# gbbin/DDP-practice

Hardware: AMD Instinct MI355X
Metric: images/sec (whole node) + 3-epoch wall-clock, MNIST ConvNet at 1/2/4/8 MI355X (higher is better)
Workload: dtype bf16; 1 GPU; model=ConvNet (2x[Conv5x5-BN-ReLU-MaxPool2] + Linear(1568,10), 29,034 params), global_batch=32, parallelism=dp1, per_rank_batch=32, impl=native (fused HIP kernels, C++ reducer/communicator), sync_bn=False, amp=autocast bf16 + GradScaler, optimizer=SGD(lr=1e-4), hipgraph=True, steps_per_graph=16, comm=none (1 rank), grad_avg=none (1 rank)

## Files before the change

### ddp_practice_amd/csrc/kernels/conv5x5.h

```cpp
#pragma once
#include "convblock_bn.h"

namespace dpa {
namespace cb {

template <int I> struct SH;
template <> struct SH<0> { static constexpr int CIN = 1, COUT = 16, H = 28, W = 28, SPLIT = 4, WROWS = 28; };
template <> struct SH<1> { static constexpr int CIN = 16, COUT = 32, H = 14, W = 14, SPLIT = 2, WROWS = 14; };

__host__ __device__ constexpr int conv5x5_win_rows(int H, int W, int nsplit, bool even) {
  const int HW = H * W, MT = (HW + 15) / 16;
  int mx = 0;
  for (int sp = 0; sp < nsplit; ++sp) {
    const int p0 = 16 * (MT * sp / nsplit), p1e = 16 * (MT * (sp + 1) / nsplit), p1 = p1e < HW ? p1e : HW;
    if (p1 <= p0) return 0;
    int lo = p0 / W - 2, hi = (p1 - 1) / W + 2;
    lo = lo < 0 ? 0 : lo;
    hi = hi > H - 1 ? H - 1 : hi;
    if (even) {
      lo &= ~1;
      hi |= 1;
    }
    mx = hi - lo + 1 > mx ? hi - lo + 1 : mx;
  }
  return mx;
}

template <typename T>
struct BwdEpi {
  const uint8_t* idx;
  const T* xh;
  float* bslab;
};

constexpr int W2F_ROWS = 32, W2F_PITCH = 424;
constexpr int W2D_ROWS = 16, W2D_PITCH = 808;
constexpr int W2F_LEN = W2F_ROWS * W2F_PITCH, W2D_LEN = W2D_ROWS * W2D_PITCH;
template <typename T>
struct WPack {
  const float* w2 = nullptr;
  T* fwd = nullptr;
  T* dgrad = nullptr;
};
template <typename T>
__device__ __forceinline__ void pack_w2(const WPack<T>& pk) {
  const int total = W2F_LEN + W2D_LEN;
  for (int e = blockIdx.x * blockDim.x + threadIdx.x; e < total; e += gridDim.x * blockDim.x) {
    if (e < W2F_LEN) {
      const int co = e / W2F_PITCH, k = e % W2F_PITCH;
      const float v = k < 400 ? pk.w2[(co * 16 + (k & 15)) * 25 + (k >> 4)] : 0.f;
      pk.fwd[e] = Cvt<T>::from_f(v);
    } else {
      const int e2 = e - W2F_LEN;
      const int ci = e2 / W2D_PITCH, k = e2 % W2D_PITCH;
      const float v = k < 800 ? pk.w2[((k & 31) * 16 + ci) * 25 + (24 - (k >> 5))] : 0.f;
      pk.dgrad[e2] = Cvt<T>::from_f(v);
    }
  }
}

struct GatherIn {
  const uint8_t* imgs = nullptr;
  const int64_t* labels = nullptr;
  const int64_t* order = nullptr;
  long long order_len = 0;
  int* ctr = nullptr;
  int64_t* lab_out = nullptr;
  float scale = 1.f, shift = 0.f;
  int nimg = 0;
};

template <typename T, int CIN, int H, int W>
__host__ __device__ constexpr size_t conv5x5_img_bytes() {
  return ((sizeof(T) * (size_t)(H + 4) * (W + 4) * CIN) + 15) / 16 * 16;
}
template <typename T, int CIN, int COUT, int H, int W>
__host__ __device__ constexpr size_t conv5x5_dyn_bytes() {
  return conv5x5_img_bytes<T, CIN, H, W>() + sizeof(T) * (size_t)COUT * (ceil_to(25 * CIN, 32) + 8);
}

template <typename T, int CIN, int COUT, int H, int W, int MODE, int PRO = 0, int EPI = 0, int WPK = 0,
          bool DYN = false, int WR = H>
__device__ __forceinline__ void
conv5x5_body(const T* __restrict__ x, const float* __restrict__ w, const float* __restrict__ bias,
             T* __restrict__ y, float* __restrict__ fslab, float* __restrict__ fstats,
             const float* __restrict__ shift, int nsplit, const PoolIn<T>& pin, const BwdIn<T>& bin,
             const BwdEpi<T>& epi, const T* __restrict__ wpk, const WPack<T>& pk, const int bid,
             const GatherIn& gin = GatherIn{}) {
  static_assert(CIN == 1 || CIN % 8 == 0, "CIN must be 1 or a multiple of 8");
  static_assert(COUT % 16 == 0, "COUT must be a multiple of 16");
  static_assert((H * W) % 4 == 0, "H*W must be a multiple of 4");
  static_assert(PRO != 2 || MODE == 2, "PRO 2 is a data-grad prologue");
  static_assert(PRO != 3 || (CIN == 1 && MODE != 2), "PRO 3 gathers single-channel input images");
  static_assert(EPI == 0 || MODE == 2, "EPI 1 is a data-grad epilogue");
  constexpr int NCH = CIN >= 8 ? CIN / 8 : 1;
  constexpr int HP = H + 4, WPD = W + 4;
  constexpr int K = 25 * CIN;
  constexpr int KP = ceil_to(K, 32);
  constexpr int KS = KP / 32;
  constexpr int KPW = KP + 8;
  constexpr int NT = COUT / 16;
  constexpr int HW = H * W;
  constexpr int MT = (HW + 15) / 16;
  typedef MM<T> mm;

  T* img;
  T* wl;
  if constexpr (DYN) {
    img = reinterpret_cast<T*>(dpa_dyn_lds);
    wl = reinterpret_cast<T*>(dpa_dyn_lds + conv5x5_img_bytes<T, CIN, H, W>());
  } else {
// ... 125 lines not shown
    }
  };
  auto store_epi = [&]() {
    if constexpr (EPI == 1) {
#pragma unroll
      for (int i = 0; i < EIT; ++i) {
        const int e = tid + i * NTHR;
        if (e < COUT * enp) {
          const int co = e / enp, pp = e % enp;
          eidx[co * EPIX + pp] = ei[i];
          exh[co * EPIX + pp] = ex[i];
        }
      }
    }
  };
  if constexpr (PRO != 2) {
    load_epi();
    store_epi();
  }
  DPA_STAMP(2);
  constexpr int DQ = PRO != 1 ? 1
                     : (CIN % 8 == 0 && sizeof(T) == 2) ? 8 * ((CIN / 8 * SR * W + NTHR - 1) / NTHR)
                                                          : (CIN * SR * W + NTHR - 1) / NTHR;
  int dq_e[DQ];
  T dq_p[DQ], dq_x[DQ];
  uint8_t dq_i[DQ];
#pragma unroll
  for (int d = 0; d < DQ; ++d) dq_e[d] = -1;
  if constexpr (PRO == 0) {
    stage_chw<T, CIN, H, W>(xb, [&](int ci, int h, int ww, T a, T bb) {
      img[imo((h + 2) * WPD + (ww + 2), ci)] = a;
      img[imo((h + 2) * WPD + (ww + 3), ci)] = bb;
    });
  } else if constexpr (PRO == 3) {
    static_assert(HW % 4 == 0 && W % 4 == 0, "4-pixel groups stay inside a row");
    constexpr int G4 = HW / 4, GIT = (G4 + NTHR - 1) / NTHR;
    const int step = __builtin_amdgcn_readfirstlane(*reinterpret_cast<volatile int*>(gin.ctr));
    long long pos = (long long)step * gin.nimg + b;
    pos = pos < gin.order_len ? pos : gin.order_len - 1;
    const int64_t src = gin.order[pos];
    const uint32_t* s4 = reinterpret_cast<const uint32_t*>(gin.imgs + src * HW);
    uint32_t v4[GIT];
#pragma unroll
    for (int i = 0; i < GIT; ++i)
      if (tid + i * NTHR < G4) v4[i] = s4[tid + i * NTHR];
    if (sp == 0 && tid == 0) gin.lab_out[b] = gin.labels[src];
// ... 31 lines not shown
    const bool wr = pin.p_out != nullptr;
    if constexpr (CIN % 8 == 0 && sizeof(T) == 2) {
      constexpr int NO = CIN / 8, NPI = NO * RP, IT8 = (NPI + NTHR - 1) / NTHR;
      P top[IT8][8], bot[IT8][8];
      auto ld8 = [&](int i, int o, int ho, int wo) {
#pragma unroll
        for (int j = 0; j < 8; ++j) {
          const P* src = reinterpret_cast<const P*>(yb + ((size_t)(8 * o + j) * 2 * H + 2 * ho) * 2 * W + 2 * wo);
          top[i][j] = src[0];
          bot[i][j] = src[W];
        }
      };
#pragma unroll
      for (int i = 0; i < IT8; ++i) {
        const int e8 = tid + i * NTHR;
        if constexpr (WIN) {
          const int ec = min(e8, NPI - 1);
          ld8(i, ec / RP, min(r_lo + (ec % RP) / W, H - 1), ec % W);
        } else if (e8 < NPI) {
          ld8(i, e8 / RP, (e8 % RP) / W, e8 % W);
        }
      }
      load_wpk();
      bn_finalize<CIN>(pin.bn, sc_s, beta_s, mean_s, istd_s, part, bid);
      DPA_STAMP(3);
#pragma unroll
      for (int i = 0; i < IT8; ++i) {
        const int e8 = tid + i * NTHR;
        const int o = e8 / RP, hl = (e8 % RP) / W, ho = r_lo + hl, wo = e8 % W;
        if (e8 < NPI && (!WIN || hl < r_n)) {
          const int pix = ho * W + wo;
          const bool own = wr && pix >= p_lo && pix < p_hi;
          unsigned pk[4];
#pragma unroll
          for (int j = 0; j < 8; ++j) {
            const int ci = 8 * o + j;
            float best, xh;
            int bi;
            bn_relu_max4x<T>(top[i][j], bot[i][j], sc_s[ci], beta_s[ci], mean_s[ci], istd_s[ci], best, bi, xh);
            const T pvj = Cvt<T>::from_f(best);
            const unsigned bits = __builtin_bit_cast(unsigned short, pvj);
            if (j & 1) pk[j >> 1] |= bits << 16; else pk[j >> 1] = bits;
            const int e = ci * HW + pix;
            const int d = i * 8 + j;
            dq_e[d] = own ? e : -1;
            dq_p[d] = pvj;
// ... 2 lines not shown
          }
          *reinterpret_cast<uint4*>(&img[imo((ho + 2) * WPD + (wo + 2), 8 * o)]) = make_uint4(pk[0], pk[1], pk[2], pk[3]);
        }
      }
    } else {
      constexpr int NPS = CIN * RP, IT = (NPS + NTHR - 1) / NTHR;
      P top[IT], bot[IT];
      auto ld1 = [&](int i, int ci, int ho, int wo) {
        const P* src = reinterpret_cast<const P*>(yb + ((size_t)ci * 2 * H + 2 * ho) * 2 * W + 2 * wo);
        top[i] = src[0];
        bot[i] = src[W];
      };
#pragma unroll
      for (int i = 0; i < IT; ++i) {
        const int e = tid + i * NTHR;
        if constexpr (WIN) {
          const int ec = min(e, NPS - 1);
          ld1(i, ec / RP, min(r_lo + (ec % RP) / W, H - 1), ec % W);
        } else if (e < NPS) {
          ld1(i, e / RP, (e % RP) / W, e % W);
        }
      }
      load_wpk();
      bn_finalize<CIN>(pin.bn, sc_s, beta_s, mean_s, istd_s, part, bid);
      DPA_STAMP(3);
#pragma unroll
      for (int i = 0; i < IT; ++i) {
        const int e = tid + i * NTHR;
        const int ci = e / RP, hl = (e % RP) / W, ho = r_lo + hl, wo = e % W;
        if (e < NPS && (!WIN || hl < r_n)) {
          const int pix = ho * W + wo;
          float best, xh;
          int bi;
          bn_relu_max4x<T>(top[i], bot[i], sc_s[ci], beta_s[ci], mean_s[ci], istd_s[ci], best, bi, xh);
          const T pv = Cvt<T>::from_f(best);
          img[imo((ho + 2) * WPD + (wo + 2), ci)] = pv;
          dq_e[i] = wr && pix >= p_lo && pix < p_hi ? ci * HW + pix : -1;
          dq_p[i] = pv;
          dq_i[i] = (uint8_t)(bi | (best > 0.f ? IDX_RELU : 0));
          dq_x[i] = Cvt<T>::from_f(xh);
        }
      }
    }
  } else {
    __shared__ float coef[5 * CIN], sums[2 * CIN];
    __shared__ float part[NTHR];
// ... 25 lines not shown
        if (WIN && h >= r_n) return;
        const int hp = r_lo + h + 2;
        img[imo(hp * WPD + (ww + 2), c)] = v00;
        img[imo(hp * WPD + (ww + 3), c)] = v01;
        img[imo((hp + 1) * WPD + (ww + 2), c)] = v10;
        img[imo((hp + 1) * WPD + (ww + 3), c)] = v11;
      });
    }
    store_epi();
  }
  DPA_STAMP(4);
  __syncthreads();
  DPA_STAMP(5);
  if constexpr (PRO == 1) {
    constexpr int NPO = CIN * HW;
#pragma unroll
    for (int d = 0; d < DQ; ++d)
      if (dq_e[d] >= 0) {
        const size_t o = (size_t)b * NPO + dq_e[d];
        pin.p_out[o] = dq_p[d];
        pin.idx_out[o] = dq_i[d];
        pin.xh_out[o] = dq_x[d];
      }
  }

  const int lane = tid & 63, wv = tid >> 6;
  const int r = lane & 15, q = lane >> 4;

  float s1[NT], s2[NT];
#pragma unroll
  for (int nt = 0; nt < NT; ++nt) s1[nt] = s2[nt] = 0.f;

  for (int mt = mt0 + wv; mt < mt1; mt += NTHR / 64) {
    const int m = mt * 16 + r;
    const int mm_ = m < HW ? m : HW - 1;
    const int oh = mm_ / W, ow = mm_ % W;
    f32x4 acc[NT];
#pragma unroll
    for (int nt = 0; nt < NT; ++nt) acc[nt] = f32x4{0.f, 0.f, 0.f, 0.f};
#pragma unroll
    for (int s = 0; s < KS; ++s) {
      typename mm::frag a;
      if constexpr (CIN == 1) {
#pragma unroll
        for (int j = 0; j < 8; ++j) {
          const int tap = 32 * s + 8 * q + j;
// ... 57 lines not shown
    if (tid < 2 * COUT) {
      float t = 0.f;
#pragma unroll
      for (int w2 = 0; w2 < NTHR / 64; ++w2) t += lstat[w2 * 2 * COUT + tid];
      row[tid] = t;
    }
    if constexpr (MODE == 0) {
      if (tid == 0) {
        const int p0 = mt0 * 16, p1 = min(mt1 * 16, HW);
        row[2 * COUT] = (float)(p1 - p0);
      }
      if (bid == 0 && tid < COUT) fstats[2 * COUT + 1 + tid] = shift[tid];
    }
  }
  DPA_STAMP(7);
}

template <typename T, int CIN, int COUT, int H, int W, int MODE, int PRO = 0, int EPI = 0, int WPK = 0, int WR = H>
__global__ void __launch_bounds__(NTHR)
conv5x5_kernel(const T* __restrict__ x, const float* __restrict__ w, const float* __restrict__ bias,
               T* __restrict__ y, float* __restrict__ fslab, float* __restrict__ fstats,
               const float* __restrict__ shift, int nsplit, PoolIn<T> pin = PoolIn<T>{},
               BwdIn<T> bin = BwdIn<T>{}, BwdEpi<T> epi = BwdEpi<T>{}, const T* __restrict__ wpk = nullptr,
               WPack<T> pk = WPack<T>{}, GatherIn gin = GatherIn{}) {
  conv5x5_body<T, CIN, COUT, H, W, MODE, PRO, EPI, WPK, false, WR>(x, w, bias, y, fslab, fstats, shift, nsplit, pin,
                                                                   bin, epi, wpk, pk, (int)blockIdx.x, gin);
}

}
}
```

### ddp_practice_amd/csrc/kernels/convnet_fused.hip

```cpp
#include <type_traits>

#include "conv5x5.h"
#include "conv5x5_wgrad.h"
#include "comm/xgmi.h"

namespace dpa {
namespace cnf {

using cb::BNParams;
using cb::bn_finalize;
using cb::bn_relu_max4x;
using cb::BwdEpi;
using cb::BwdIn;
using cb::IDX_POS;
using cb::IDX_RELU;
using cb::Pair2;
using cb::PoolIn;
using cb::with_t;

constexpr int HF = 256;
constexpr int NTHR_HB = 256;

template <typename T, int C, int H, int W, int NMAX>
__global__ void __launch_bounds__(HF)
// ... 175 lines not shown
  bi.dbeta = dbeta.has_value() ? dbeta->data_ptr<float>() : nullptr;
  return bi;
}

typedef std::shared_ptr<xgmi::XgmiComm> XcPtr;
static xgmi::XSite site_of(const XcPtr& xc, int s) { return xc ? xc->site(s) : xgmi::XSite{}; }

int64_t fwd2_split(bool fp32) { return fp32 ? cb::kFwd2SplitT<float> : cb::kFwd2SplitT<__half>; }

template <int NSPLIT, bool EVEN>
constexpr int conv2_wr() {
  constexpr int need = cb::conv5x5_win_rows(14, 14, NSPLIT, EVEN);
  static_assert(need > 0, "conv2: more workgroups per image than 16-pixel tiles");
  return need < 14 ? need : 14;
}
static void conv2_row_window(int wr, int nsplit, bool even, const char* what) {
  const int need = cb::conv5x5_win_rows(14, 14, nsplit, even);
  TORCH_CHECK(need > 0 && (wr >= 14 || need <= wr), what, ": a split in ", nsplit, " stages up to ", need,
              " rows, the kernel's window holds ", wr);
}
template <typename T>
constexpr int kFwd2WR = conv2_wr<cb::kFwd2SplitT<T>, false>();

void conv2_fwd(at::Tensor y1, c10::optional<at::Tensor> fslab1, at::Tensor fstats1, at::Tensor g1, at::Tensor b1,
               at::Tensor rm1, at::Tensor rv1, at::Tensor nbt1, double momentum, double eps, bool train, at::Tensor w2,
               at::Tensor bias2, at::Tensor y2, c10::optional<at::Tensor> fslab2, at::Tensor fstats2, at::Tensor rm2,
               c10::optional<at::Tensor> p1_out, c10::optional<at::Tensor> idx1_out,
               c10::optional<at::Tensor> xh1_out, at::Tensor wpk, XcPtr xc) {
  DPA_CHECK_INPUT(y1); DPA_CHECK_INPUT(w2); DPA_CHECK_INPUT(y2); DPA_CHECK_INPUT(wpk);
  TORCH_CHECK(wpk.numel() == cb::W2F_LEN && wpk.scalar_type() == y1.scalar_type(), "packed conv2 weights");
  const int B = (int)y1.size(0);
  TORCH_CHECK(y1.size(1) == 16 && y1.size(2) == 28 && y1.size(3) == 28 && w2.size(0) == 32 && w2.size(1) == 16,
              "fused conv2 expects the ConvNet shapes");
  TORCH_CHECK(y2.scalar_type() == y1.scalar_type());
  TORCH_CHECK(p1_out.has_value() == idx1_out.has_value() && p1_out.has_value() == xh1_out.has_value());
  if (p1_out.has_value())
    TORCH_CHECK(p1_out->numel() == (int64_t)B * 16 * 196 && idx1_out->numel() == p1_out->numel() &&
                xh1_out->numel() == p1_out->numel());
  const int ns = fwd2_split(y1.scalar_type() == at::kFloat);
  if (train) TORCH_CHECK(fslab2.has_value() && fslab2->numel() == (int64_t)B * ns * cb::fslab_row(32));
  if (B == 0) return;
  BNParams bp = bn_params(fslab1, fstats1, g1, b1, rm1, rv1, nbt1, momentum, eps, train, 16);
  if (train) {
    bp.xs = site_of(xc, xgmi::kSiteFwd1);
    xgmi::set_site_grid(bp.xs, B * ns, "conv2_fwd");
  }
  hipStream_t stream = cur_stream();
  with_t(dt_of(y1), [&](auto tag) {
    typedef decltype(tag) T;
    PoolIn<T> pin{dptr<T>(y1), bp, p1_out.has_value() ? dptr<T>(*p1_out) : nullptr,
                  idx1_out.has_value() ? idx1_out->data_ptr<uint8_t>() : nullptr,
                  xh1_out.has_value() ? dptr<T>(*xh1_out) : nullptr};
    constexpr int WR = kFwd2WR<T>;
    conv2_row_window(WR, ns, false, "conv2_fwd");
    if (train)
      hipLaunchKernelGGL((cb::conv5x5_kernel<T, 16, 32, 14, 14, 0, 1, 0, 1, WR>), dim3(B * ns), dim3(cb::NTHR), 0,
                         stream, nullptr, nullptr, bias2.data_ptr<float>(), dptr<T>(y2), fslab2->data_ptr<float>(),
                         fstats2.data_ptr<float>(), rm2.data_ptr<float>(), ns, pin, BwdIn<T>{}, BwdEpi<T>{},
                         dptr<T>(wpk), cb::WPack<T>{});
    else
      hipLaunchKernelGGL((cb::conv5x5_kernel<T, 16, 32, 14, 14, 1, 1, 0, 1, WR>), dim3(B * ns), dim3(cb::NTHR), 0,
                         stream, nullptr, nullptr, bias2.data_ptr<float>(), dptr<T>(y2), nullptr, nullptr, nullptr,
                         ns, pin, BwdIn<T>{}, BwdEpi<T>{}, dptr<T>(wpk), cb::WPack<T>{});
  });
  DPA_CHECK_LAUNCH();
}

void head_fwd(at::Tensor y2, c10::optional<at::Tensor> fslab2, at::Tensor fstats2, at::Tensor g2, at::Tensor b2,
              at::Tensor rm2, at::Tensor rv2, at::Tensor nbt2, double momentum, double eps, bool train, at::Tensor wfc,
              at::Tensor bfc, at::Tensor logits, c10::optional<at::Tensor> p2_out, c10::optional<at::Tensor> idx2_out,
              c10::optional<at::Tensor> xh2_out, XcPtr xc) {
  DPA_CHECK_INPUT(y2); DPA_CHECK_INPUT(wfc); DPA_CHECK_INPUT(logits);
  const int B = (int)y2.size(0), N = (int)wfc.size(0);
  TORCH_CHECK(y2.size(1) == 32 && y2.size(2) == 14 && y2.size(3) == 14 && wfc.size(1) == 32 * 49,
              "fused head expects the ConvNet shapes");
  TORCH_CHECK(N >= 1 && N <= 64, "fused head supports up to 64 classes");
  TORCH_CHECK(logits.numel() == (int64_t)B * N && logits.scalar_type() == y2.scalar_type());
  TORCH_CHECK(p2_out.has_value() == idx2_out.has_value() && p2_out.has_value() == xh2_out.has_value());
  if (p2_out.has_value())
    TORCH_CHECK(p2_out->numel() == (int64_t)B * 1568 && idx2_out->numel() == p2_out->numel() &&
                xh2_out->numel() == p2_out->numel());
  if (B == 0) return;
// ... 528 lines not shown
        B * fwd2_split(std::is_same<T, float>::value));
    ok = ok && co_resident(reinterpret_cast<const void*>(&head_fwd_kernel<T, 32, 14, 14, 16>), (int)B, HF, 0) &&
         co_resident(reinterpret_cast<const void*>(&head_fwd_kernel<T, 32, 14, 14, 64>), (int)B, HF, 0);
    chk(reinterpret_cast<const void*>(&cb::conv5x5_kernel<T, 32, 16, 14, 14, 2, 2, 1, 1, kDgrad2WR<T>>), B * kDgradSplitT<T>);
    if (conv2_bwd_dyn<T>())
      ok = ok && co_resident(reinterpret_cast<const void*>(&conv2_bwd_dyn_kernel<T>),
                             (int)(B * kDgradSplitT<T> + wgrad2_wgs(B) + FC_BLOCKS), cb::NTHR,
                             conv2_bwd_dyn_bytes<T>());
    else if constexpr (!std::is_same<T, float>::value)
      chk(reinterpret_cast<const void*>(&conv2_bwd_kernel<T>), B * kDgradSplitT<T> + wgrad2_wgs(B) + FC_BLOCKS);
    chk(reinterpret_cast<const void*>(&conv2_wgrad_kernel<T>), wgrad2_wgs(B));
    chk(reinterpret_cast<const void*>(&cb::conv5x5_wgrad_kernel<T, 1, 16, 28, 28, WG1_ROWS, 2>),
        wgrad_bn_rows(1, B));
    chk(reinterpret_cast<const void*>(&wgrad1_slab2_kernel<T>), wgrad_bn_rows(1, B));
  });
  return ok;
}

}

void register_convnet_fused(pybind11::module& m) {
  namespace py = pybind11;
  auto s = m.def_submodule("convnet", "whole-ConvNet fused kernels");
  s.def("conv2_fwd", &cnf::conv2_fwd);
  s.def("head_fwd", &cnf::head_fwd);
  s.def("head_bwd", &cnf::head_bwd);
  s.def("head_bwd_lds", &cnf::head_bwd_lds);
  s.def("dgrad2_rows", &cnf::dgrad2_rows, py::arg("B"), py::arg("fp32") = false);
  s.def("conv1_fwd_pack", &cnf::conv1_fwd_pack);
  s.def("conv1_fwd_pack_gather", &cnf::conv1_fwd_pack_gather);
#ifdef DPA_TIMING
  s.def("read_stamps", []() {
    auto out = at::empty({DPA_MAX_STAMP_BLOCKS, DPA_NSTAMPS}, at::TensorOptions().dtype(at::kLong));
    DPA_CHECK_HIP(hipDeviceSynchronize());
    DPA_CHECK_HIP(hipMemcpyFromSymbol(out.data_ptr(), HIP_SYMBOL(dpa_stamps), sizeof(unsigned long long) *
                                      DPA_MAX_STAMP_BLOCKS * DPA_NSTAMPS));
    return out;
  });
  s.def("clear_stamps", []() {
    DPA_CHECK_HIP(hipDeviceSynchronize());
    std::vector<unsigned long long> z(DPA_MAX_STAMP_BLOCKS * DPA_NSTAMPS, 0ull);
    DPA_CHECK_HIP(hipMemcpyToSymbol(HIP_SYMBOL(dpa_stamps), z.data(), z.size() * sizeof(unsigned long long)));
  });
#endif
  s.attr("W2F_LEN") = cb::W2F_LEN;
  s.attr("W2D_LEN") = cb::W2D_LEN;
  s.def("conv2_dgrad", &cnf::conv2_dgrad);
// ... 11 lines not shown
```

### ddp_practice_amd/csrc/kernels/convnet_head.hip

```cpp
#include <cstdlib>

#include "comm/xgmi.h"
#include "convblock_bn.h"

namespace dpa {
namespace cnh {

using cb::BNParams;
using cb::IDX_RELU;
using cb::Pair2;

constexpr int NT_MAX = 1024;
constexpr int C = 32, H = 14, W = 14, HO = 7, WO = 7, PP = 49, K = C * PP;
constexpr int BMAX = 64;
constexpr int NMAX = 16;

constexpr int kArrShift = 57, kBadShift = 50;
constexpr unsigned long long kSumMask = (1ull << kBadShift) - 1ull;
constexpr double kFix = 16777216.0;
constexpr float kRowMax = 1048575.f;

struct HeadRow {
  const int64_t* target;
  int64_t ignore_index;
  float smoothing;
  const float* scale;
  int has_scale;
  unsigned long long* state;
  float* loss;
  float* dlog;
  void* dls;
  void* dp2;
  float* bsum;
  int* chk;
};



template <typename T, int NM, int NT>
__global__ void __launch_bounds__(NT)
head_row_kernel(const T* __restrict__ y, BNParams bn, const float* __restrict__ wfc, const float* __restrict__ bfc,
                T* __restrict__ logits, T* __restrict__ p_out, uint8_t* __restrict__ idx_out,
                T* __restrict__ xh_out, int B, int N, HeadRow hr) {
  typedef typename Pair2<T>::type P;
  constexpr int IT = (K + NT - 1) / NT;
  constexpr int NW = NT / 64;
  constexpr int CL = NT / C;
  __shared__ float sc_s[C], beta_s[C], mean_s[C], istd_s[C];
  __shared__ float part_s[NT];
  __shared__ float red[NW][NM];
  __shared__ float lgs[NM];
  __shared__ float gs[2][IT * NT];

  const int tid = threadIdx.x, b = blockIdx.x;
  const int lane = tid & 63, wv = tid >> 6;

  DPA_STAMP(0);
  const T* yb = y + (size_t)b * C * H * W;
  P top[IT], bot[IT];
#pragma unroll
  for (int i = 0; i < IT; ++i) {
    const int k = min(tid + i * NT, K - 1);
    const int c = k / PP, j = k % PP, ho = j / WO, wo = j % WO;
    const P* src = reinterpret_cast<const P*>(yb + ((size_t)c * H + 2 * ho) * W + 2 * wo);
    top[i] = src[0];
    bot[i] = src[W / 2];
  }
  float wq[NM][IT];
#pragma unroll
  for (int n = 0; n < NM; ++n) {
    const float* wr = wfc + (size_t)min(n, N - 1) * K;
#pragma unroll
    for (int i = 0; i < IT; ++i) wq[n][i] = wr[min(tid + i * NT, K - 1)];
  }
  float bias[NM];
#pragma unroll
  for (int n = 0; n < NM; ++n) bias[n] = bfc[min(n, N - 1)];
  const int64_t tgt_lane = hr.target[min(lane, B - 1)];
  const int64_t tgt = hr.target[b];
  const float scv = hr.scale[0];
  DPA_STAMP(1);
  constexpr int RU = NT == 256 && cb::kFwd2SplitT<T> > 2 ? (32 * cb::kFwd2SplitT<T> + 2) / 3 : cb::RSUM_U;
  cb::bn_finalize<C, RU>(bn, sc_s, beta_s, mean_s, istd_s, part_s, b);
  DPA_STAMP(2);
  if (hr.chk != nullptr && b == 0 && tid == 0) {
    hr.chk[0] = 0;
    hr.chk[1] = __float_as_int(scv);
  }
  float pf[IT], xf[IT];
  uint8_t ixr[IT];
#pragma unroll
  for (int i = 0; i < IT; ++i) {
    const int k = tid + i * NT;
    const int c = min(k, K - 1) / PP;
    float best, xh;
    int bi;
    cb::bn_relu_max4x<T>(top[i], bot[i], sc_s[c], beta_s[c], mean_s[c], istd_s[c], best, bi, xh);
    const T pv = Cvt<T>::from_f(best);
    const T xq = Cvt<T>::from_f(xh);
    ixr[i] = (uint8_t)(bi | (best > 0.f ? IDX_RELU : 0));
    pf[i] = k < K ? Cvt<T>::to_f(pv) : 0.f;
    xf[i] = Cvt<T>::to_f(xq);
    if (k < K) {
      const size_t o = (size_t)b * K + k;
      p_out[o] = pv;
      idx_out[o] = ixr[i];
      xh_out[o] = xq;
    }
  }
#pragma unroll
  for (int n = 0; n < NM; ++n)
#pragma unroll
    for (int i = 0; i < IT; ++i) wq[n][i] = n < N ? rnd_t<T>(wq[n][i]) : 0.f;
#pragma unroll
  for (int n = 0; n < NM; ++n) {
    float a = 0.f;
#pragma unroll
    for (int i = 0; i < IT; ++i) a += pf[i] * wq[n][i];
    a = wave_sum_dpp(a);
    if (lane == 0) red[wv][n] = a;
  }
  lds_barrier();
  if (NW > 4) {
    if (tid < NM) {
      float t = 0.f;
#pragma unroll
      for (int n = 0; n < NM; ++n) t = tid == n ? bias[n] : t;
#pragma unroll
      for (int w = 0; w < NW; ++w) t += red[w][tid];
      lgs[tid] = t;
    }
    lds_barrier();
  }
  DPA_STAMP(3);
  float lg[NM];
  float mx = -INFINITY, sx = 0.f, xt = 0.f;
// ... 95 lines not shown
      const float l = (cnt > 0.f && bad == 0) ? (float)(sum / (double)cnt) : NAN;
      hr.loss[0] = l;
      if (hr.has_scale) hr.loss[1] = l * scv;
      __hip_atomic_store(hr.state, 0ull, __ATOMIC_RELAXED, __HIP_MEMORY_SCOPE_AGENT);
    }
  }
}

template <typename F>
static void with_t(DT dt, F&& f) {
  switch (dt) {
    case DT::F32: f(float{}); break;
    case DT::BF16: f(__hip_bfloat16{}); break;
    case DT::F16: f(__half{}); break;
  }
}

bool supported(int64_t B, int64_t N) { return B >= 1 && B <= BMAX && N >= 1 && N <= NMAX; }

bool resident(at::ScalarType st) {
  bool ok = true;
  with_t(dt_of(at::empty({0}, at::TensorOptions().dtype(st))), [&](auto tag) {
    typedef decltype(tag) T;
    ok = co_resident(reinterpret_cast<const void*>(&head_row_kernel<T, 10, NT_MAX>), BMAX, NT_MAX, 0) &&
         co_resident(reinterpret_cast<const void*>(&head_row_kernel<T, NMAX, 256>), BMAX, 256, 0);
  });
  return ok;
}

void head_step(at::Tensor y2, at::Tensor fslab2, at::Tensor fstats2, at::Tensor g2, at::Tensor b2, at::Tensor rm2,
               at::Tensor rv2, at::Tensor nbt2, double momentum, double eps, at::Tensor wfc, at::Tensor bfc,
               at::Tensor logits, at::Tensor p2, at::Tensor idx2, at::Tensor xh2, at::Tensor target,
               int64_t ignore_index, double smoothing, c10::optional<at::Tensor> scale, at::Tensor state,
               at::Tensor loss, at::Tensor dlog, c10::optional<at::Tensor> dls, c10::optional<at::Tensor> dp2,
               c10::optional<at::Tensor> bsum_rows, std::shared_ptr<xgmi::XgmiComm> xc,
               c10::optional<at::Tensor> chk) {
  DPA_CHECK_INPUT(y2); DPA_CHECK_INPUT(wfc); DPA_CHECK_INPUT(logits); DPA_CHECK_INPUT(p2); DPA_CHECK_INPUT(target);
  DPA_CHECK_INPUT(bfc); DPA_CHECK_INPUT(idx2); DPA_CHECK_INPUT(xh2); DPA_CHECK_INPUT(dlog);
  const int B = (int)y2.size(0), N = (int)wfc.size(0);
  TORCH_CHECK(y2.size(1) == C && y2.size(2) == H && y2.size(3) == W && wfc.size(1) == K, "head_step: ConvNet shapes");
  TORCH_CHECK(supported(B, N), "head_step: B <= ", BMAX, " and N <= ", NMAX);
  TORCH_CHECK(bfc.numel() == N && wfc.scalar_type() == at::kFloat && bfc.scalar_type() == at::kFloat);
  TORCH_CHECK(logits.numel() == (int64_t)B * N && logits.scalar_type() == y2.scalar_type());
  TORCH_CHECK(p2.numel() == (int64_t)B * K && idx2.numel() == p2.numel() && xh2.numel() == p2.numel());
  TORCH_CHECK(p2.scalar_type() == y2.scalar_type() && xh2.scalar_type() == y2.scalar_type() &&
              idx2.scalar_type() == at::kByte);
  TORCH_CHECK(target.scalar_type() == at::kLong && target.numel() == B);
  TORCH_CHECK(state.numel() >= 1 && state.scalar_type() == at::kLong && state.is_cuda());
  TORCH_CHECK(loss.numel() >= 2 && loss.scalar_type() == at::kFloat && loss.is_cuda());
  TORCH_CHECK(dlog.numel() == (int64_t)B * N && dlog.scalar_type() == at::kFloat);
  TORCH_CHECK(scale.has_value() == dls.has_value(), "head_step: scale and dls go together");
  const bool bwd = dp2.has_value();
  TORCH_CHECK(bwd == bsum_rows.has_value(), "head_step: dp2 and bsum_rows go together");
  if (scale.has_value()) {
    DPA_CHECK_INPUT(*scale); DPA_CHECK_INPUT(*dls);
    TORCH_CHECK(scale->numel() >= 1 && scale->scalar_type() == at::kFloat);
    TORCH_CHECK(dls->numel() == (int64_t)B * N && dls->scalar_type() == y2.scalar_type());
  }
  if (bwd) {
// ... 25 lines not shown
  hr.smoothing = (float)smoothing;
  hr.scale = scale.has_value() ? scale->data_ptr<float>() : loss.data_ptr<float>();
  hr.has_scale = scale.has_value() ? 1 : 0;
  hr.chk = nullptr;
  if (chk.has_value()) {
    DPA_CHECK_INPUT(*chk);
    TORCH_CHECK(chk->scalar_type() == at::kInt && chk->numel() == 2 && scale.has_value(),
                "head_step: gradient-check words need the scaler's scale and int32[2]");
    hr.chk = chk->data_ptr<int>();
  }
  hr.state = reinterpret_cast<unsigned long long*>(state.data_ptr<int64_t>());
  hr.loss = loss.data_ptr<float>();
  hr.dlog = dlog.data_ptr<float>();
  hr.dls = dls.has_value() ? dls->data_ptr() : nullptr;
  hr.dp2 = bwd ? dp2->data_ptr() : nullptr;
  hr.bsum = bwd ? bsum_rows->data_ptr<float>() : nullptr;
  with_t(dt_of(y2), [&](auto tag) {
    typedef decltype(tag) T;
    static const int nt = [] {
      const char* e = std::getenv("DPA_HEAD_NT");
      return e != nullptr && std::atoi(e) == NT_MAX ? NT_MAX : 256;
    }();
    const int ntl = N <= 10 ? nt : 256;
    auto kern = N > 10 ? head_row_kernel<T, NMAX, 256>
                       : (nt == 256 ? head_row_kernel<T, 10, 256> : head_row_kernel<T, 10, NT_MAX>);
    hipLaunchKernelGGL(kern, dim3(B), dim3(ntl), 0, cur_stream(), dptr<T>(y2), bp, wfc.data_ptr<float>(),
                       bfc.data_ptr<float>(), dptr<T>(logits), dptr<T>(p2), idx2.data_ptr<uint8_t>(), dptr<T>(xh2), B,
                       N, hr);
  });
  DPA_CHECK_LAUNCH();
}

}

void register_convnet_head(pybind11::module& m) {
  auto s = m.def_submodule("convnet_head", "ConvNet head: forward + loss + backward in one launch");
  s.def("head_step", &cnh::head_step);
  s.def("supported", &cnh::supported);
  s.def("resident", &cnh::resident);
  DPA_DEF_STAMP_FNS(s);
  s.attr("C") = cnh::C;
  s.attr("NMAX") = cnh::NMAX;
}

}
```

### ddp_practice_amd/ops/convnet_fused.py

```python
from __future__ import annotations

import os

import torch

from .._ext import load as _load_ext


def _mods():
    C = _load_ext()
    return C.convblock, C.convnet


def supported(model, x: torch.Tensor) -> bool:
    if not x.is_cuda or x.dim() != 4 or tuple(x.shape[1:]) != (1, 28, 28):
        return False
    l1, l2, fc = model.layer1, model.layer2, model.fc
    for seq, cin, cout in ((l1, 1, 16), (l2, 16, 32)):
        conv, bn = seq[0], seq[1]
        if (conv.in_channels, conv.out_channels, conv.kernel_size, conv.stride, conv.padding) != \
                (cin, cout, (5, 5), (1, 1), (2, 2)) or conv.bias is None or conv.groups != 1:
            return False
        if not (bn.track_running_stats and bn.affine):
            return False
# ... 11 lines not shown
def _fused_site_engine(comm, batch: int, dtype: torch.dtype):
    flag = os.environ.get("DPA_FUSED_SYNC")
    if flag == "0":
        return None
    if flag != "1" and os.environ.get("DPA_SHARED_GPU") == "1" and getattr(comm, "world_size", 1) > 2:
        return None
    xc = getattr(comm, "xgmi", None)
    if xc is None:
        return None
    key = (batch, dtype)
    if key not in _RESIDENT:
        _RESIDENT[key] = bool(_load_ext().convnet.sites_resident(batch, dtype))
    return xc if _RESIDENT[key] else None


class PreCE:

    __slots__ = ("target", "ignore_index", "smoothing", "scale", "loss", "dlog", "dls")

    def __init__(self, target, ignore_index, smoothing, scale, loss, dlog, dls):
        self.target, self.ignore_index, self.smoothing = target, ignore_index, smoothing
        self.scale, self.loss, self.dlog, self.dls = scale, loss, dlog, dls


_HEAD_OK: dict = {}
_HEAD_SPEC = os.environ.get("DPA_HEAD_SPEC", "1") != "0"


def _head_step_ok(B: int, N: int, dtype: torch.dtype) -> bool:
    if os.environ.get("DPA_HEAD_STEP", "1") == "0":
        return False
    H = _load_ext().convnet_head
    if not H.supported(B, N):
        return False
    if dtype not in _HEAD_OK:
        _HEAD_OK[dtype] = bool(H.resident(dtype))
    return _HEAD_OK[dtype]


class ConvNetFn(torch.autograd.Function):
    @staticmethod
    def forward(ctx, x, w1, b1, g1, be1, w2, b2, g2, be2, wfc, bfc, bufs, training, moms, epss, comm, cdtype,
                labels=None, ce_cfg=(-100, 0.0), holder=None, state=None, gather=None, sink=None):
        cb, cn = _mods()
        rm1, rv1, nbt1, rm2, rv2, nbt2 = bufs
        m1, m2 = (-1.0 if m is None else float(m) for m in moms)
# ... 9 lines not shown
        logits = torch.empty((B, N), dtype=cdtype, device=dev)
        wpk_f = torch.empty(cn.W2F_LEN, dtype=cdtype, device=dev)
        wpk_d = torch.empty(cn.W2D_LEN, dtype=cdtype, device=dev)
        fstats1 = torch.empty(cb.stats_len(16), dtype=torch.float32, device=dev)
        fstats2 = torch.empty(cb.stats_len(32), dtype=torch.float32, device=dev)
        if training:
            fslab1 = torch.empty(cb.fwd_rows(1, 16, 28, 28, B) * cb.fslab_row(16), dtype=torch.float32, device=dev)
            fslab2 = torch.empty(B * cn.fwd2_split(cdtype == torch.float32) * cb.fslab_row(32), dtype=torch.float32,
                                 device=dev)
            p1 = torch.empty((B, 16, 14, 14), dtype=cdtype, device=dev)
            idx1 = torch.empty((B, 16, 14, 14), dtype=torch.uint8, device=dev)
            xh1 = torch.empty((B, 16, 14, 14), dtype=cdtype, device=dev)
            p2 = torch.empty((B, 32 * 49), dtype=cdtype, device=dev)
            idx2 = torch.empty((B, 32 * 49), dtype=torch.uint8, device=dev)
            xh2 = torch.empty((B, 32 * 49), dtype=cdtype, device=dev)
            if gather is not None:
                imgs, lbls, order, ctr, lab_out, gsc, gsh = gather
                cn.conv1_fwd_pack_gather(x, w1, b1, y1, fslab1, fstats1, rm1, w2, wpk_f, wpk_d, imgs, lbls, order,
                                         ctr, lab_out, gsc, gsh)
            else:
                cn.conv1_fwd_pack(x, w1, b1, y1, fslab1, fstats1, rm1, w2, wpk_f, wpk_d)
            if sync and xc is None:
                comm.all_reduce_(fslab1)
            cn.conv2_fwd(y1, fslab1, fstats1, g1, be1, rm1, rv1, nbt1, m1, e1, True, w2, b2, y2, fslab2, fstats2,
                         rm2, p1, idx1, xh1, wpk_f, xc)
            if sync and xc is None:
                comm.all_reduce_(fslab2)
            ctx.spec = None
            ctx.chk = ctx.chk_scale = None
            if labels is not None and state is not None and _head_step_ok(B, N, cdtype):
                from .head import seed_scale

                scale = seed_scale(dev) if _HEAD_SPEC else None
                f32 = dict(dtype=torch.float32, device=dev)
                loss_buf = torch.empty(2, **f32)
                dlog = torch.empty((B, N), **f32)
                dls = torch.empty((B, N), dtype=cdtype, device=dev) if scale is not None else None
                spec = None
                if scale is not None:
                    dp2 = torch.empty_like(p2)
                    bsum2 = torch.empty(B * 64, **f32)
                    spec = (dls, dp2, bsum2)
                    from .head import _UNIT

                    ddp = getattr(sink, "_deferred_ddp", None) if sink is not None else None
                    ddp_world = int(ddp[1].world_size) if ddp is not None and ddp[1] is not None else 1
                    chk = None
                    if (sink is not None and _PRECHECK and scale is not _UNIT.get(dev)
                            and (xc is not None or (not sync and ddp_world == 1))
                            and hasattr(sink, "set_prechecked")):
                        sink.clear_prechecked()
                        chk = sink.grad_chk(2, dev)
                    ctx.chk, ctx.chk_scale = chk, (scale if chk is not None else None)
                    _load_ext().convnet_head.head_step(
                        y2, fslab2, fstats2, g2, be2, rm2, rv2, nbt2, m2, e2, wfc, bfc, logits, p2, idx2, xh2, labels,
                        int(ce_cfg[0]), float(ce_cfg[1]), scale, state, loss_buf, dlog, dls, dp2, bsum2, xc, chk)
                else:
                    _load_ext().convnet_head.head_step(
                        y2, fslab2, fstats2, g2, be2, rm2, rv2, nbt2, m2, e2, wfc, bfc, logits, p2, idx2, xh2, labels,
                        int(ce_cfg[0]), float(ce_cfg[1]), None, state, loss_buf, dlog, None, None, None, xc, None)
                ctx.spec = spec
                if holder is not None:
                    holder["ce"] = PreCE(labels, int(ce_cfg[0]), float(ce_cfg[1]), scale, loss_buf, dlog, dls)
            else:
                cn.head_fwd(y2, fslab2, fstats2, g2, be2, rm2, rv2, nbt2, m2, e2, True, wfc, bfc, logits, p2, idx2,
                            xh2, xc)
            ctx.save_for_backward(x, wpk_d, wfc, g1, g2, y1, p1, idx1, xh1, fstats1, y2, p2, idx2, xh2, fstats2)
        else:
            cn.conv1_fwd_pack(x, w1, b1, y1, None, None, None, w2, wpk_f, wpk_d)
            cn.conv2_fwd(y1, None, fstats1, g1, be1, rm1, rv1, nbt1, m1, e1, False, w2, b2, y2, None, fstats2, rm2,
                         None, None, None, wpk_f, None)
            cn.head_fwd(y2, None, fstats2, g2, be2, rm2, rv2, nbt2, m2, e2, False, wfc, bfc, logits, None, None,
                        None, None)
        ctx.training = training
        ctx.sink = sink
        ctx.w1b1 = (w1, b1) if sink is not None else None
        ctx.allp = (w1, b1, g1, be1, w2, b2, g2, be2, wfc, bfc) if sink is not None else None
        ctx.sync = sync
        ctx.comm = comm
        ctx.xc = xc
        ctx.eps = (e1, e2)
        ctx.shapes = (w1.shape, w2.shape, wfc.shape)
        return logits
# ... 126 lines not shown
```

Baseline: 788,000 images/s.

## Pre-pack FC weights to bf16 in conv2 forward for coalesced head loads

```diff
diff --git a/ddp_practice_amd/csrc/kernels/conv5x5.h b/ddp_practice_amd/csrc/kernels/conv5x5.h
--- a/ddp_practice_amd/csrc/kernels/conv5x5.h
+++ b/ddp_practice_amd/csrc/kernels/conv5x5.h
@@ -1,5 +1,6 @@
 #pragma once
 #include "convblock_bn.h"
+#include "fc_pack.h"
 
 namespace dpa {
 namespace cb {
@@ -42,6 +43,25 @@
   T* fwd = nullptr;
   T* dgrad = nullptr;
 };
+template <typename T>
+struct FcPack {
+  const float* wfc = nullptr;
+  T* fcp = nullptr;
+  int fc_n = 0, fc_nm = 0;
+  int fc_lanes = 0;
+};
+template <typename T>
+__device__ __forceinline__ float fc_pack_load(const FcPack<T>& pk, int s) {
+  const int src = fcp::src_of<(int)sizeof(T)>(min(s, fcp::len(pk.fc_nm, sizeof(T)) - 1), pk.fc_nm, pk.fc_n);
+  const float v = pk.wfc[max(src, 0)];
+  return src >= 0 ? v : 0.f;
+}
+template <typename T>
+__device__ __forceinline__ void fc_pack_store(const FcPack<T>& pk, int s, float v0) {
+  const int total = fcp::len(pk.fc_nm, sizeof(T));
+  if (s < total) pk.fcp[s] = Cvt<T>::from_f(v0);
+  for (s += pk.fc_lanes; s < total; s += pk.fc_lanes) pk.fcp[s] = Cvt<T>::from_f(fc_pack_load<T>(pk, s));
+}
 template <typename T>
 __device__ __forceinline__ void pack_w2(const WPack<T>& pk) {
   const int total = W2F_LEN + W2D_LEN;
@@ -86,7 +106,7 @@
              T* __restrict__ y, float* __restrict__ fslab, float* __restrict__ fstats,
              const float* __restrict__ shift, int nsplit, const PoolIn<T>& pin, const BwdIn<T>& bin,
              const BwdEpi<T>& epi, const T* __restrict__ wpk, const WPack<T>& pk, const int bid,
-             const GatherIn& gin = GatherIn{}) {
+             const GatherIn& gin = GatherIn{}, const FcPack<T>& fcj = FcPack<T>{}) {
   static_assert(CIN == 1 || CIN % 8 == 0, "CIN must be 1 or a multiple of 8");
   static_assert(COUT % 16 == 0, "COUT must be a multiple of 16");
   static_assert((H * W) % 4 == 0, "H*W must be a multiple of 4");
@@ -258,6 +278,8 @@
   constexpr int DQ = PRO != 1 ? 1
                      : (CIN % 8 == 0 && sizeof(T) == 2) ? 8 * ((CIN / 8 * SR * W + NTHR - 1) / NTHR)
                                                           : (CIN * SR * W + NTHR - 1) / NTHR;
+  const bool fc_job = PRO == 1 && fcj.fcp != nullptr;
+  float fc_v = 0.f;
   int dq_e[DQ];
   T dq_p[DQ], dq_x[DQ];
   uint8_t dq_i[DQ];
@@ -335,6 +357,7 @@
         }
       }
       load_wpk();
+      if (fc_job) fc_v = fc_pack_load<T>(fcj, bid * NTHR + tid);
       bn_finalize<CIN>(pin.bn, sc_s, beta_s, mean_s, istd_s, part, bid);
       DPA_STAMP(3);
 #pragma unroll
@@ -383,6 +406,7 @@
         }
       }
       load_wpk();
+      if (fc_job) fc_v = fc_pack_load<T>(fcj, bid * NTHR + tid);
       bn_finalize<CIN>(pin.bn, sc_s, beta_s, mean_s, istd_s, part, bid);
       DPA_STAMP(3);
 #pragma unroll
@@ -454,6 +478,7 @@
         pin.idx_out[o] = dq_i[d];
         pin.xh_out[o] = dq_x[d];
       }
+    if (fc_job) fc_pack_store<T>(fcj, bid * NTHR + tid, fc_v);
   }
 
   const int lane = tid & 63, wv = tid >> 6;
@@ -557,10 +582,10 @@
                T* __restrict__ y, float* __restrict__ fslab, float* __restrict__ fstats,
                const float* __restrict__ shift, int nsplit, PoolIn<T> pin = PoolIn<T>{},
                BwdIn<T> bin = BwdIn<T>{}, BwdEpi<T> epi = BwdEpi<T>{}, const T* __restrict__ wpk = nullptr,
-               WPack<T> pk = WPack<T>{}, GatherIn gin = GatherIn{}) {
+               WPack<T> pk = WPack<T>{}, GatherIn gin = GatherIn{}, FcPack<T> fcj = FcPack<T>{}) {
   conv5x5_body<T, CIN, COUT, H, W, MODE, PRO, EPI, WPK, false, WR>(x, w, bias, y, fslab, fstats, shift, nsplit, pin,
-                                                                   bin, epi, wpk, pk, (int)blockIdx.x, gin);
-}
-
-}
-}
+                                                                   bin, epi, wpk, pk, (int)blockIdx.x, gin, fcj);
+}
+
+}
+}
diff --git a/ddp_practice_amd/csrc/kernels/convnet_fused.hip b/ddp_practice_amd/csrc/kernels/convnet_fused.hip
--- a/ddp_practice_amd/csrc/kernels/convnet_fused.hip
+++ b/ddp_practice_amd/csrc/kernels/convnet_fused.hip
@@ -221,11 +221,18 @@
 template <typename T>
 constexpr int kFwd2WR = conv2_wr<cb::kFwd2SplitT<T>, false>();
 
+int fc_pack_nm(int64_t N) { return N < 1 || N > 16 ? 0 : (N <= 10 ? 10 : 16); }
+int64_t fc_pack_len(int64_t N, int64_t itemsize) {
+  TORCH_CHECK(fc_pack_nm(N) > 0 && (itemsize == 2 || itemsize == 4), "fc pack: N <= 16, 2- or 4-byte elements");
+  return fcp::len(fc_pack_nm(N), (int)itemsize);
+}
+
 void conv2_fwd(at::Tensor y1, c10::optional<at::Tensor> fslab1, at::Tensor fstats1, at::Tensor g1, at::Tensor b1,
                at::Tensor rm1, at::Tensor rv1, at::Tensor nbt1, double momentum, double eps, bool train, at::Tensor w2,
                at::Tensor bias2, at::Tensor y2, c10::optional<at::Tensor> fslab2, at::Tensor fstats2, at::Tensor rm2,
                c10::optional<at::Tensor> p1_out, c10::optional<at::Tensor> idx1_out,
-               c10::optional<at::Tensor> xh1_out, at::Tensor wpk, XcPtr xc) {
+               c10::optional<at::Tensor> xh1_out, at::Tensor wpk, XcPtr xc, c10::optional<at::Tensor> wfc,
+               c10::optional<at::Tensor> fcpk) {
   DPA_CHECK_INPUT(y1); DPA_CHECK_INPUT(w2); DPA_CHECK_INPUT(y2); DPA_CHECK_INPUT(wpk);
   TORCH_CHECK(wpk.numel() == cb::W2F_LEN && wpk.scalar_type() == y1.scalar_type(), "packed conv2 weights");
   const int B = (int)y1.size(0);
@@ -238,6 +245,18 @@
                 xh1_out->numel() == p1_out->numel());
   const int ns = fwd2_split(y1.scalar_type() == at::kFloat);
   if (train) TORCH_CHECK(fslab2.has_value() && fslab2->numel() == (int64_t)B * ns * cb::fslab_row(32));
+  TORCH_CHECK(wfc.has_value() == fcpk.has_value() && (train || !fcpk.has_value()),
+              "conv2_fwd: the fc pack needs wfc and fcpk, in training");
+  int fc_n = 0, fc_nm = 0;
+  if (fcpk.has_value()) {
+    DPA_CHECK_INPUT(*wfc); DPA_CHECK_INPUT(*fcpk);
+    fc_n = (int)wfc->size(0);
+    fc_nm = fc_pack_nm(fc_n);
+    TORCH_CHECK(wfc->dim() == 2 && wfc->size(1) == fcp::K && wfc->scalar_type() == at::kFloat && fc_nm > 0,
+                "conv2_fwd: fc weights [N <= 16][1568] f32");
+    TORCH_CHECK(fcpk->scalar_type() == y1.scalar_type() && fcpk->numel() == fc_pack_len(fc_n, y1.element_size()),
+                "conv2_fwd: fc pack size");
+  }
   if (B == 0) return;
   BNParams bp = bn_params(fslab1, fstats1, g1, b1, rm1, rv1, nbt1, momentum, eps, train, 16);
   if (train) {
@@ -252,11 +271,19 @@
                   xh1_out.has_value() ? dptr<T>(*xh1_out) : nullptr};
     constexpr int WR = kFwd2WR<T>;
     conv2_row_window(WR, ns, false, "conv2_fwd");
+    cb::FcPack<T> pk{};
+    if (fcpk.has_value()) {
+      pk.wfc = wfc->data_ptr<float>();
+      pk.fcp = dptr<T>(*fcpk);
+      pk.fc_n = fc_n;
+      pk.fc_nm = fc_nm;
+      pk.fc_lanes = B * ns * cb::NTHR;
+    }
     if (train)
       hipLaunchKernelGGL((cb::conv5x5_kernel<T, 16, 32, 14, 14, 0, 1, 0, 1, WR>), dim3(B * ns), dim3(cb::NTHR), 0,
                          stream, nullptr, nullptr, bias2.data_ptr<float>(), dptr<T>(y2), fslab2->data_ptr<float>(),
                          fstats2.data_ptr<float>(), rm2.data_ptr<float>(), ns, pin, BwdIn<T>{}, BwdEpi<T>{},
-                         dptr<T>(wpk), cb::WPack<T>{});
+                         dptr<T>(wpk), cb::WPack<T>{}, cb::GatherIn{}, pk);
     else
       hipLaunchKernelGGL((cb::conv5x5_kernel<T, 16, 32, 14, 14, 1, 1, 0, 1, WR>), dim3(B * ns), dim3(cb::NTHR), 0,
                          stream, nullptr, nullptr, bias2.data_ptr<float>(), dptr<T>(y2), nullptr, nullptr, nullptr,
@@ -831,7 +858,12 @@
 void register_convnet_fused(pybind11::module& m) {
   namespace py = pybind11;
   auto s = m.def_submodule("convnet", "whole-ConvNet fused kernels");
-  s.def("conv2_fwd", &cnf::conv2_fwd);
+  s.def("conv2_fwd", &cnf::conv2_fwd, py::arg("y1"), py::arg("fslab1"), py::arg("fstats1"), py::arg("g1"),
+        py::arg("b1"), py::arg("rm1"), py::arg("rv1"), py::arg("nbt1"), py::arg("momentum"), py::arg("eps"),
+        py::arg("train"), py::arg("w2"), py::arg("bias2"), py::arg("y2"), py::arg("fslab2"), py::arg("fstats2"),
+        py::arg("rm2"), py::arg("p1_out"), py::arg("idx1_out"), py::arg("xh1_out"), py::arg("wpk"), py::arg("xc"),
+        py::arg("wfc") = py::none(), py::arg("fcpk") = py::none());
+  s.def("fc_pack_len", &cnf::fc_pack_len, py::arg("N"), py::arg("itemsize"));
   s.def("head_fwd", &cnf::head_fwd);
   s.def("head_bwd", &cnf::head_bwd);
   s.def("head_bwd_lds", &cnf::head_bwd_lds);
diff --git a/ddp_practice_amd/csrc/kernels/convnet_head.hip b/ddp_practice_amd/csrc/kernels/convnet_head.hip
--- a/ddp_practice_amd/csrc/kernels/convnet_head.hip
+++ b/ddp_practice_amd/csrc/kernels/convnet_head.hip
@@ -2,6 +2,7 @@
 
 #include "comm/xgmi.h"
 #include "convblock_bn.h"
+#include "fc_pack.h"
 
 namespace dpa {
 namespace cnh {
@@ -37,11 +38,12 @@
 
 
 
-template <typename T, int NM, int NT>
+template <typename T, int NM, int NT, bool PK = false>
 __global__ void __launch_bounds__(NT)
 head_row_kernel(const T* __restrict__ y, BNParams bn, const float* __restrict__ wfc, const float* __restrict__ bfc,
                 T* __restrict__ logits, T* __restrict__ p_out, uint8_t* __restrict__ idx_out,
-                T* __restrict__ xh_out, int B, int N, HeadRow hr) {
+                T* __restrict__ xh_out, int B, int N, HeadRow hr, const T* __restrict__ wpk = nullptr) {
+  static_assert(!PK || (NT == fcp::NT && K == fcp::K), "the fc pack is laid out for the 256-lane head");
   typedef typename Pair2<T>::type P;
   constexpr int IT = (K + NT - 1) / NT;
   constexpr int NW = NT / 64;
@@ -67,11 +69,19 @@
     bot[i] = src[W / 2];
   }
   float wq[NM][IT];
-#pragma unroll
-  for (int n = 0; n < NM; ++n) {
-    const float* wr = wfc + (size_t)min(n, N - 1) * K;
-#pragma unroll
-    for (int i = 0; i < IT; ++i) wq[n][i] = wr[min(tid + i * NT, K - 1)];
+  constexpr int EPC = fcp::epc(sizeof(T)), NCH = PK ? fcp::nch(NM, sizeof(T)) : 1;
+  uint4 wch[NCH];
+  if constexpr (PK) {
+    const uint4* src = reinterpret_cast<const uint4*>(wpk) + tid;
+#pragma unroll
+    for (int j = 0; j < NCH; ++j) wch[j] = src[j * NT];
+  } else {
+#pragma unroll
+    for (int n = 0; n < NM; ++n) {
+      const float* wr = wfc + (size_t)min(n, N - 1) * K;
+#pragma unroll
+      for (int i = 0; i < IT; ++i) wq[n][i] = wr[min(tid + i * NT, K - 1)];
+    }
   }
   float bias[NM];
 #pragma unroll
@@ -111,7 +121,19 @@
 #pragma unroll
   for (int n = 0; n < NM; ++n)
 #pragma unroll
-    for (int i = 0; i < IT; ++i) wq[n][i] = n < N ? rnd_t<T>(wq[n][i]) : 0.f;
+    for (int i = 0; i < IT; ++i) {
+      if constexpr (PK) {
+        const int r = n * IT + i, wi = (r % EPC) * (int)sizeof(T) / 4;
+        const uint4 c = wch[r / EPC];
+        const unsigned w32 = wi == 0 ? c.x : wi == 1 ? c.y : wi == 2 ? c.z : c.w;
+        if constexpr (sizeof(T) == 4)
+          wq[n][i] = __uint_as_float(w32);
+        else
+          wq[n][i] = Cvt<T>::to_f(__builtin_bit_cast(T, (unsigned short)((r & 1) ? w32 >> 16 : w32 & 0xffffu)));
+      } else {
+        wq[n][i] = n < N ? rnd_t<T>(wq[n][i]) : 0.f;
+      }
+    }
 #pragma unroll
   for (int n = 0; n < NM; ++n) {
     float a = 0.f;
@@ -253,8 +275,9 @@
   bool ok = true;
   with_t(dt_of(at::empty({0}, at::TensorOptions().dtype(st))), [&](auto tag) {
     typedef decltype(tag) T;
-    ok = co_resident(reinterpret_cast<const void*>(&head_row_kernel<T, 10, NT_MAX>), BMAX, NT_MAX, 0) &&
-         co_resident(reinterpret_cast<const void*>(&head_row_kernel<T, NMAX, 256>), BMAX, 256, 0);
+    ok = co_resident(reinterpret_cast<const void*>(&head_row_kernel<T, 10, NT_MAX, false>), BMAX, NT_MAX, 0) &&
+         co_resident(reinterpret_cast<const void*>(&head_row_kernel<T, NMAX, 256, false>), BMAX, 256, 0) &&
+         co_resident(reinterpret_cast<const void*>(&head_row_kernel<T, NMAX, 256, true>), BMAX, 256, 0);
   });
   return ok;
 }
@@ -265,7 +288,7 @@
                int64_t ignore_index, double smoothing, c10::optional<at::Tensor> scale, at::Tensor state,
                at::Tensor loss, at::Tensor dlog, c10::optional<at::Tensor> dls, c10::optional<at::Tensor> dp2,
                c10::optional<at::Tensor> bsum_rows, std::shared_ptr<xgmi::XgmiComm> xc,
-               c10::optional<at::Tensor> chk) {
+               c10::optional<at::Tensor> chk, c10::optional<at::Tensor> fcpk) {
   DPA_CHECK_INPUT(y2); DPA_CHECK_INPUT(wfc); DPA_CHECK_INPUT(logits); DPA_CHECK_INPUT(p2); DPA_CHECK_INPUT(target);
   DPA_CHECK_INPUT(bfc); DPA_CHECK_INPUT(idx2); DPA_CHECK_INPUT(xh2); DPA_CHECK_INPUT(dlog);
   const int B = (int)y2.size(0), N = (int)wfc.size(0);
@@ -337,11 +360,21 @@
       return e != nullptr && std::atoi(e) == NT_MAX ? NT_MAX : 256;
     }();
     const int ntl = N <= 10 ? nt : 256;
-    auto kern = N > 10 ? head_row_kernel<T, NMAX, 256>
-                       : (nt == 256 ? head_row_kernel<T, 10, 256> : head_row_kernel<T, 10, NT_MAX>);
+    const bool pk = fcpk.has_value() && ntl == 256;
+    const T* wpk = nullptr;
+    if (pk) {
+      DPA_CHECK_INPUT(*fcpk);
+      TORCH_CHECK(fcpk->scalar_type() == y2.scalar_type() &&
+                      fcpk->numel() == fcp::len(N > 10 ? NMAX : 10, sizeof(T)),
+                  "head_step: fc pack size (convnet.fc_pack_len)");
+      wpk = dptr<T>(*fcpk);
+    }
+    auto kern = N > 10 ? (pk ? head_row_kernel<T, NMAX, 256, true> : head_row_kernel<T, NMAX, 256, false>)
+                : nt == 256 ? (pk ? head_row_kernel<T, 10, 256, true> : head_row_kernel<T, 10, 256, false>)
+                            : head_row_kernel<T, 10, NT_MAX, false>;
     hipLaunchKernelGGL(kern, dim3(B), dim3(ntl), 0, cur_stream(), dptr<T>(y2), bp, wfc.data_ptr<float>(),
                        bfc.data_ptr<float>(), dptr<T>(logits), dptr<T>(p2), idx2.data_ptr<uint8_t>(), dptr<T>(xh2), B,
-                       N, hr);
+                       N, hr, wpk);
   });
   DPA_CHECK_LAUNCH();
 }
@@ -350,7 +383,13 @@
 
 void register_convnet_head(pybind11::module& m) {
   auto s = m.def_submodule("convnet_head", "ConvNet head: forward + loss + backward in one launch");
-  s.def("head_step", &cnh::head_step);
+  namespace py = pybind11;
+  s.def("head_step", &cnh::head_step, py::arg("y2"), py::arg("fslab2"), py::arg("fstats2"), py::arg("g2"),
+        py::arg("b2"), py::arg("rm2"), py::arg("rv2"), py::arg("nbt2"), py::arg("momentum"), py::arg("eps"),
+        py::arg("wfc"), py::arg("bfc"), py::arg("logits"), py::arg("p2"), py::arg("idx2"), py::arg("xh2"),
+        py::arg("target"), py::arg("ignore_index"), py::arg("smoothing"), py::arg("scale"), py::arg("state"),
+        py::arg("loss"), py::arg("dlog"), py::arg("dls"), py::arg("dp2"), py::arg("bsum_rows"), py::arg("xc"),
+        py::arg("chk"), py::arg("fcpk") = py::none());
   s.def("supported", &cnh::supported);
   s.def("resident", &cnh::resident);
   DPA_DEF_STAMP_FNS(s);
diff --git a/ddp_practice_amd/csrc/kernels/fc_pack.h b/ddp_practice_amd/csrc/kernels/fc_pack.h
--- /dev/null
+++ b/ddp_practice_amd/csrc/kernels/fc_pack.h
@@ -0,0 +1,27 @@
+#pragma once
+#include "common.h"
+
+namespace dpa {
+namespace fcp {
+
+constexpr int K = 32 * 49;
+constexpr int NT = 256;
+constexpr int IT = (K + NT - 1) / NT;
+
+__host__ __device__ constexpr int epc(int itemsize) { return 16 / itemsize; }
+__host__ __device__ constexpr int nch(int nm, int itemsize) {
+  return (nm * IT + epc(itemsize) - 1) / epc(itemsize);
+}
+__host__ __device__ constexpr int len(int nm, int itemsize) { return nch(nm, itemsize) * NT * epc(itemsize); }
+
+template <int ITEM>
+__device__ __forceinline__ int src_of(int s, int nm, int N) {
+  constexpr int E = epc(ITEM);
+  const int chunk = s / E, e = s % E;
+  const int j = chunk / NT, t = chunk % NT;
+  const int r = j * E + e, n = r / IT, i = r % IT, k = t + i * NT;
+  return (n < nm && n < N && k < K) ? n * K + k : -1;
+}
+
+}
+}
diff --git a/ddp_practice_amd/ops/convnet_fused.py b/ddp_practice_amd/ops/convnet_fused.py
--- a/ddp_practice_amd/ops/convnet_fused.py
+++ b/ddp_practice_amd/ops/convnet_fused.py
@@ -57,6 +57,8 @@
         self.target, self.ignore_index, self.smoothing = target, ignore_index, smoothing
         self.scale, self.loss, self.dlog, self.dls = scale, loss, dlog, dls
 
+
+_FC_PACK = os.environ.get("DPA_FC_PACK", "1") != "0"
 
 _HEAD_OK: dict = {}
 _HEAD_SPEC = os.environ.get("DPA_HEAD_SPEC", "1") != "0"
@@ -112,13 +114,17 @@
                 cn.conv1_fwd_pack(x, w1, b1, y1, fslab1, fstats1, rm1, w2, wpk_f, wpk_d)
             if sync and xc is None:
                 comm.all_reduce_(fslab1)
+            head_step = labels is not None and state is not None and _head_step_ok(B, N, cdtype)
+            fcpk = None
+            if head_step and _FC_PACK and cdtype != torch.float32:
+                fcpk = torch.empty(cn.fc_pack_len(N, y1.element_size()), dtype=cdtype, device=dev)
             cn.conv2_fwd(y1, fslab1, fstats1, g1, be1, rm1, rv1, nbt1, m1, e1, True, w2, b2, y2, fslab2, fstats2,
-                         rm2, p1, idx1, xh1, wpk_f, xc)
+                         rm2, p1, idx1, xh1, wpk_f, xc, wfc if fcpk is not None else None, fcpk)
             if sync and xc is None:
                 comm.all_reduce_(fslab2)
             ctx.spec = None
             ctx.chk = ctx.chk_scale = None
-            if labels is not None and state is not None and _head_step_ok(B, N, cdtype):
+            if head_step:
                 from .head import seed_scale
 
                 scale = seed_scale(dev) if _HEAD_SPEC else None
@@ -144,11 +150,11 @@
                     ctx.chk, ctx.chk_scale = chk, (scale if chk is not None else None)
                     _load_ext().convnet_head.head_step(
                         y2, fslab2, fstats2, g2, be2, rm2, rv2, nbt2, m2, e2, wfc, bfc, logits, p2, idx2, xh2, labels,
-                        int(ce_cfg[0]), float(ce_cfg[1]), scale, state, loss_buf, dlog, dls, dp2, bsum2, xc, chk)
+                        int(ce_cfg[0]), float(ce_cfg[1]), scale, state, loss_buf, dlog, dls, dp2, bsum2, xc, chk, fcpk)
                 else:
                     _load_ext().convnet_head.head_step(
                         y2, fslab2, fstats2, g2, be2, rm2, rv2, nbt2, m2, e2, wfc, bfc, logits, p2, idx2, xh2, labels,
-                        int(ce_cfg[0]), float(ce_cfg[1]), None, state, loss_buf, dlog, None, None, None, xc, None)
+                        int(ce_cfg[0]), float(ce_cfg[1]), None, state, loss_buf, dlog, None, None, None, xc, None, fcpk)
                 ctx.spec = spec
                 if holder is not None:
                     holder["ce"] = PreCE(labels, int(ce_cfg[0]), float(ce_cfg[1]), scale, loss_buf, dlog, dls)
```

New measurement: 792,600 images/s, median of 6. No clear change (+0.6%).
